# DylanAuty/ObjCAViT

Hardware: AMD Instinct MI355X
Metric: images/sec (640x480, bs=16) forward depth inference, 3 batches of 16 in flight per GPU; AbsRel vs CPU ref (higher is better)
Workload: dtype f32 (fp16 / bf16 split contractions)

## Files before the change

include/objcavit_hip.h:

```cpp
#ifndef OBJCAVIT_HIP_H
#define OBJCAVIT_HIP_H

#include <stddef.h>
#include <stdint.h>

#ifdef __cplusplus
extern "C" {
#endif

typedef void* ocv_stream_t;

#define OCV_ABI_VERSION 5
int ocv_abi_version(void);
const char* ocv_last_error(void);

int ocv_range_flag_set(unsigned* flag);
int ocv_range_flag_take_fwd(unsigned* flag, unsigned* out, ocv_stream_t stream);
int ocv_attention_set_fp32_range(int on);
int ocv_attention_set_dispatch(int form);

#define OCV_ACT_NONE 0
#define OCV_ACT_RELU 1
#define OCV_ACT_LEAKY_RELU 2
#define OCV_ACT_SILU 3
// ... 133 lines not shown
int ocv_pointwise_conv_nhwc_split_ws_fwd(const float* x, const float* gate, int rows_per_image, const void* w_packed,
                                         const float* bias, const float* residual, float* y, void* y_hl, long M, int Cin, int Cout,
                                         int act, void* workspace, size_t workspace_bytes, ocv_stream_t stream);
int ocv_pointwise_hl_set_dispatch(int rt, int tn);
int ocv_pointwise_hl_fwd(const void* x_hl, int Cin, const void* w_packed, long w_image_elems, int rows_per_image,
                         const float* bias, const float* residual, float* y, void* y_hl, long M, int Cout, int act,
                         ocv_stream_t stream);
int ocv_stem_conv_fwd(const float* x, const float* w, const float* bias, float* y, int B, int Cin, int H, int W, int Cout,
                      int k, int stride, int pad_t, int pad_l, int Ho, int Wo, int act, ocv_stream_t stream);
int ocv_depthwise_conv_nhwc_fwd(const float* in, const float* w, const float* bias, float* out, int B, int C, int H,
                                int W, int k, int stride, int pad_t, int pad_l, int Ho, int Wo, int act,
                                ocv_stream_t stream);
int ocv_depthwise_set_dispatch(int mode);
int ocv_depthwise_sum_tiles(int B, int C, int Ho, int Wo, int k, int stride);
int ocv_depthwise_conv_nhwc_sum_fwd(const float* in, const float* w, const float* bias, float* out, float* part, int B,
                                    int C, int H, int W, int k, int stride, int pad_t, int pad_l, int Ho, int Wo,
                                    ocv_stream_t stream);
int ocv_se_gate_partials_fwd(const float* part, int tiles, long pixels_per_image, const float* w1, const float* b1,
                             const float* w2t, const float* b2, float* gate, float* hidden_ws, int B, int C, int R,
                             ocv_stream_t stream);
int ocv_depthwise_conv_nhwc_sum_hl_fwd(const float* in, const float* w, const float* bias, float* out, void* out_hl, float* part,
                                       int B, int C, int H, int W, int k, int stride, int pad_t, int pad_l, int Ho, int Wo,
                                       ocv_stream_t stream);
int ocv_se_gate_weights_fwd(const float* part, int tiles, long pixels_per_image, const float* w1, const float* b1,
                            const float* w2t, const float* b2, const float* W, void* w_packed, long w_image_elems, float* gate,
                            float* hidden_ws, int B, int C, int R, int N, ocv_stream_t stream);


size_t ocv_channel_mean_workspace_bytes(int B, int C, long P);
int ocv_channel_mean_nhwc_fwd(const float* x, float* out, int B, int C, long P, void* workspace, size_t workspace_bytes,
                              ocv_stream_t stream);

int ocv_se_gate_fwd(const float* mean, const float* w1, const float* b1, const float* w2t, const float* b2, float* gate,
                    float* hidden_ws, int B, int C, int R, ocv_stream_t stream);

int ocv_conv_nhwc_fwd(const float* x1, int C1, const float* x2, int C2, const void* w_hi, const void* w_lo,
                      const float* bias, const float* residual, float* y, int B, int H, int W, int Cout, int ksize,
                      int act, ocv_stream_t stream);
int ocv_conv_nhwc_exact_fwd(const float* x1, int C1, const float* x2, int C2, const float* w_tap_major, const float* bias,
                            const float* residual, float* y, int B, int H, int W, int Cout, int ksize, int act,
                            ocv_stream_t stream);
int ocv_conv3x3_nhwc_strided_fwd(const float* x, int Cin, const void* w_hi, const void* w_lo, const float* bias,
                                 const float* residual, float* y, int B, int H, int W, int Cout, int stride, int pad_t,
                                 int pad_l, int Ho, int Wo, int act, ocv_stream_t stream);

int ocv_mbconv_expand_dw_tiles(int Ho, int Wo, int k, int stride);
// ... 146 lines not shown
```

objcavit_amd/_lib.py:

```python
from __future__ import annotations

import ctypes as C
import os
from typing import Optional

_HERE = os.path.dirname(os.path.abspath(__file__))
LIB_PATH = os.environ.get("OCV_LIB_PATH") or os.path.join(_HERE, "lib", "libobjcavit_hip.so")

_f32p = C.c_void_p
_u8p = C.c_void_p
_stream = C.c_void_p
ABI_VERSION = 5


class EncoderLayerParams(C.Structure):
    _fields_ = [("struct_size", C.c_size_t)] + [(n, C.c_void_p) for n in (
        "in_proj_w", "in_proj_b", "out_proj_w", "out_proj_b", "norm1_w", "norm1_b",
        "linear1_w", "linear1_b", "linear2_w", "linear2_b", "norm2_w", "norm2_b",
        "in_proj_p3", "out_proj_p3", "linear1_p3", "linear2_p3",
        "in_proj_h2", "out_proj_h2", "linear1_h2", "linear2_h2")]

    def __init__(self, *a, **kw):
        super().__init__(*a, **kw)
        self.struct_size = C.sizeof(EncoderLayerParams)
# ... 60 lines not shown
                                          _f32p, C.c_int, C.c_int, C.c_int, C.c_int, _stream]),
    "ocv_patch_embed_workspace_bytes": (C.c_size_t, [C.c_int, C.c_int, C.c_int, C.c_int, C.c_int]),
    "ocv_patch_embed_split_workspace_bytes": (C.c_size_t, [C.c_int, C.c_int, C.c_int, C.c_int, C.c_int]),
    "ocv_patch_embed_split_fwd": (C.c_int, [C.c_void_p, C.c_int, C.c_void_p, C.c_void_p, _f32p, C.c_int, _f32p, _f32p, C.c_long, _f32p, C.c_int,
                                            C.c_int, C.c_int, C.c_int, C.c_void_p, C.c_size_t, _stream]),
    "ocv_patch_embed_fwd": (C.c_int, [_f32p, C.c_int, _f32p, _f32p, _f32p, C.c_long, _f32p, C.c_int, C.c_int, C.c_int, C.c_int,
                                      C.c_int, C.c_void_p, C.c_size_t, _stream]),
    "ocv_pixel_dot_fwd": (C.c_int, [_f32p, C.c_int, _f32p, C.c_long, C.c_int, _f32p, C.c_int, C.c_int, C.c_int, C.c_int, _stream]),
    "ocv_bin_head_workspace_bytes": (C.c_size_t, [C.c_int, C.c_int, C.c_int]),
    "ocv_bin_head_fold_fwd": (C.c_int, [_f32p, C.c_long, C.c_int, _f32p, _f32p, C.c_int, C.c_int, C.c_int, C.c_int, _stream]),
    "ocv_bin_head_folded_fwd": (C.c_int, [_f32p, C.c_int, _f32p, _f32p, _f32p, _f32p, C.c_int, C.c_int, C.c_int, C.c_int, _stream]),
    "ocv_bin_head_partials_bytes": (C.c_size_t, [C.c_int, C.c_int]),
    "ocv_bin_head_folded_ws_fwd": (C.c_int, [_f32p, C.c_int, _f32p, _f32p, _f32p, _f32p, C.c_int, C.c_int, C.c_int, C.c_int,
                                             C.c_void_p, C.c_size_t, _stream]),
    "ocv_bin_head_stats_partials_bytes": (C.c_size_t, [C.c_int, C.c_int]),
    "ocv_bin_head_folded_stats_fwd": (C.c_int, [_f32p, C.c_int, _f32p, _f32p, _f32p, _f32p, C.c_int, C.c_int, C.c_int, C.c_int,
                                                C.c_void_p, C.c_size_t, _f32p, _f32p, _stream]),
    "ocv_bin_head_fwd": (C.c_int, [_f32p, C.c_int, _f32p, C.c_long, C.c_int, _f32p, _f32p, _f32p, _f32p, C.c_int, C.c_int,
                                   C.c_int, C.c_int, C.c_int, C.c_void_p, C.c_size_t, _stream]),
    "ocv_depthwise_conv_fwd": (C.c_int, [_f32p, _f32p, _f32p, _f32p] + [C.c_int] * 11 + [_stream]),
    "ocv_depthwise_set_dispatch": (C.c_int, [C.c_int]),
    "ocv_depthwise_sum_tiles": (C.c_int, [C.c_int] * 6),
    "ocv_depthwise_conv_nhwc_sum_fwd": (C.c_int, [_f32p] * 5 + [C.c_int] * 10 + [_stream]),
    "ocv_se_gate_partials_fwd": (C.c_int, [_f32p, C.c_int, C.c_long, _f32p, _f32p, _f32p, _f32p, _f32p, _f32p, C.c_int,
                                           C.c_int, C.c_int, _stream]),
    "ocv_depth_metrics_workspace_bytes": (C.c_size_t, [C.c_int] * 3),
    "ocv_depth_metrics_fwd": (C.c_int, [_f32p, _f32p, C.c_int, C.c_int, _f32p, C.c_int, C.c_int, C.c_float, C.c_float] + [C.c_int] * 4 +
                              [C.c_long, _f32p, C.c_int, C.c_void_p, C.c_size_t, _stream]),
    "ocv_depth_metrics_loss_workspace_bytes": (C.c_size_t, [C.c_int] * 4),
    "ocv_depth_metrics_loss_fwd": (C.c_int, [_f32p, _f32p, C.c_int, C.c_int, _f32p, C.c_int, C.c_int, C.c_float, C.c_float] + [C.c_int] * 4 +
                                   [_f32p, C.c_int, C.c_long, _f32p, _f32p, C.c_int, C.c_void_p, C.c_size_t, _stream]),
    "ocv_frame_ingest_fwd": (C.c_int, [_u8p, C.c_long, C.c_long, C.c_int, C.c_int, C.c_int, C.c_int, _f32p, _f32p, C.c_int, C.c_int, C.c_int,
                                       C.c_int, C.c_long, _stream]),
    "ocv_depth_ingest_fwd": (C.c_int, [C.c_void_p, C.c_long, C.c_long, C.c_int, C.c_int, C.c_int, C.c_int, C.c_float, _f32p, C.c_int, C.c_int,
                                       C.c_int, _stream]),
    "ocv_frame_resize_supported": (C.c_int, [C.c_int] * 4),
    "ocv_frame_resize_ingest": (C.c_int, [_u8p, C.c_long, C.c_long] + [C.c_int] * 6 + [_f32p, C.c_void_p, _f32p, C.c_int, C.c_void_p, _f32p,
                                          C.c_int, _f32p, C.c_int, C.c_int, C.c_int, C.c_int, C.c_long, _stream]),
    "ocv_frame_ingest_format": (C.c_int, [C.c_int] + [_u8p, C.c_long, C.c_long] * 3 + [C.c_void_p] + [C.c_int] * 4 + [_f32p, _f32p, C.c_int,
                                          C.c_int, C.c_int, C.c_int, C.c_long, _stream]),
    "ocv_frame_resize_ingest_format": (C.c_int, [C.c_int] + [_u8p, C.c_long, C.c_long] * 3 + [C.c_void_p] + [C.c_int] * 6 +
                                       [_f32p, C.c_void_p, _f32p, C.c_int, C.c_void_p, _f32p, C.c_int, _f32p, C.c_int, C.c_int, C.c_int,
                                        C.c_int, C.c_long, _stream]),
    "ocv_frames_to_rgb24": (C.c_int, [C.c_int] + [_u8p, C.c_long, C.c_long] * 3 + [C.c_void_p] + [C.c_int] * 4 + [_u8p, C.c_int, C.c_int,
                                      C.c_int, _stream]),
    "ocv_depth_finalize_fwd": (C.c_int, [_f32p, _f32p, C.c_int, C.c_int, C.c_float, C.c_float, C.c_int, C.c_int, _f32p, C.c_void_p, C.c_float,
# ... 110 lines not shown
```

objcavit_amd/build.py:

```python
from __future__ import annotations

import os
import shutil
import subprocess
import sys

HERE = os.path.dirname(os.path.abspath(__file__))
CSRC = os.environ.get("OCV_CSRC_DIR") or os.path.join(HERE, "csrc")
LIB_DIR = os.path.join(HERE, "lib")
LIB_PATH = os.path.join(LIB_DIR, "libobjcavit_hip.so")
SOURCES = ("capi.hip", "linear.hip", "attention.hip", "patch_embed.hip", "bin_head.hip", "depthwise.hip", "conv_igemm.hip", "conv_dma.hip", "conv_winograd.hip", "encoder_nhwc.hip", "upsample.hip", "pointwise_split.hip", "stem.hip", "depthwise_se.hip", "se_gate.hip", "metrics.hip", "mbconv_fused.hip", "pos_sample.hip", "conv_exact.hip", "token_split3.hip", "xattn_split3.hip", "token_pack.hip", "tap_interp.hip", "pointwise_hl.hip", "xattn_h2.hip", "conv_few.hip", "token_h2.hip", "objects_pad.hip", "bin_edges.hip", "frame_ingest.hip", "frame_resize.hip", "depth_finalize.hip", "object_depth.hip", "point_cloud.hip", "surface_normals.hip", "object_metrics.hip", "object_frontend.hip")
ARCH = "gfx950"


def _hipcc() -> str:
    for c in (os.environ.get("HIPCC"), shutil.which("hipcc"), "/opt/rocm/bin/hipcc"):
        if c and os.path.exists(c):
            return c
    raise RuntimeError("hipcc not found")


def _stale() -> bool:
    if not os.path.exists(LIB_PATH):
        return True
    t = os.path.getmtime(LIB_PATH)
    deps = [os.path.join(CSRC, f) for f in os.listdir(CSRC)] + [os.path.join(HERE, "..", "include", "objcavit_hip.h")]
    return any(os.path.getmtime(d) > t for d in deps)


def build(force: bool = False, verbose: bool = False, out: str = None) -> str:
    out = out or os.environ.get("OCV_LIB_OUT")
    if out:
        return _build_to(os.path.abspath(out), os.path.abspath(out) + ".objs", verbose)
    if not force and not _stale():
# ... 39 lines not shown
```

objcavit_amd/csrc/depthwise_se.hip:

```cpp
#include <stdlib.h>

#include "mbconv_tile.hpp"

namespace {

struct DWSArgs {
  const float *in, *w, *bias;
  float *out, *part;
  __bf16* out_hl;
  int C, H, W, Ho, Wo, pad_t, pad_l;
  int QL, PL, RY;
  int wox, nwork, tiles, chunks;
};

template <int K, int S, int PX>
__global__ __launch_bounds__(256, 2) void dw_slide_kernel(DWSArgs p) {
  constexpr int NIN = (PX - 1) * S + K;
  constexpr bool WLDS = K > 3;
  __shared__ float4 red[256];
  __shared__ float4 wsh[WLDS ? K * K * 64 : 1];
  const int tid = threadIdx.x;
  const int q = tid % p.QL, pl = tid / p.QL;
  const int c4n = p.C >> 2;
  int tile, chunk;
// ... 335 lines not shown
template <int S, int QLP>
int launch_dwr(const DWRArgs& a, int B, hipStream_t st) {
  ocv_allow_dynamic_lds<dw_rows_kernel<S, QLP>>();
  constexpr size_t lds = DWRShape<S, QLP>::LDS;
  hipLaunchKernelGGL((dw_rows_kernel<S, QLP>), dim3((unsigned)((long)a.tiles * a.chunks * B)), dim3(dwr_threads(S)), lds, st, a);
  OCV_CHECK_LAUNCH("ocv_depthwise_conv_nhwc_sum_fwd(rows)");
  return 0;
}

}

extern "C" int ocv_depthwise_set_dispatch(int mode) {
  OCV_CHECK_ARG(mode >= 0 && mode <= 2, "ocv_depthwise_set_dispatch: mode must be 0 (automatic), 1 (register window) or 2 (LDS rows), got %d", mode);
  dw_dispatch() = mode;
  return 0;
}

extern "C" int ocv_depthwise_sum_tiles(int B, int C, int Ho, int Wo, int k, int stride) {
  if (B < 1 || C < 4 || C % 4 != 0 || Ho < 1 || Wo < 1 || (k != 3 && k != 5) || (stride != 1 && stride != 2)) return 0;
  if (dw_use_rows(C, Ho, Wo, k, stride)) return dwr_geom(B, C, Ho, Wo, stride).tiles;
  return dws_geom(B, C, Ho, Wo, k, stride).tiles;
}

extern "C" int ocv_depthwise_conv_nhwc_sum_fwd(const float* in, const float* w, const float* bias, float* out, float* part,
                                               int B, int C, int H, int W, int k, int stride, int pad_t, int pad_l,
                                               int Ho, int Wo, ocv_stream_t stream) {
  return ocv_depthwise_conv_nhwc_sum_hl_fwd(in, w, bias, out, nullptr, part, B, C, H, W, k, stride, pad_t, pad_l, Ho, Wo, stream);
}

extern "C" int ocv_depthwise_conv_nhwc_sum_hl_fwd(const float* in, const float* w, const float* bias, float* out, void* out_hl,
                                                  float* part, int B, int C, int H, int W, int k, int stride, int pad_t,
                                                  int pad_l, int Ho, int Wo, ocv_stream_t stream) {
  OCV_CHECK_ARG(in && w && (out || out_hl) && part, "ocv_depthwise_conv_nhwc_sum_fwd: null pointer");
  OCV_CHECK_ARG(out_hl == nullptr || (C % 32 == 0 && ocv_aligned16(out_hl)), "ocv_depthwise_conv_nhwc_sum_hl_fwd: the split output needs C to be a multiple of 32 (got %d) and 16-byte alignment", C);
  if (ocv_check_dw_geometry("ocv_depthwise_conv_nhwc_sum_fwd", true, B, C, H, W, k, stride, pad_t, pad_l, Ho, Wo,
                            ocv_aligned16(in) && ocv_aligned16(w) && ocv_aligned16(out) && ocv_aligned16(bias) && ocv_aligned16(part)) != 0)
    return -1;
  hipStream_t st = (hipStream_t)stream;
  if (dw_use_rows(C, Ho, Wo, k, stride)) {
    const DWRGeom r = dwr_geom(B, C, Ho, Wo, stride);
    OCV_CHECK_ARG((long)r.tiles * r.chunks * B < (1L << 31), "ocv_depthwise_conv_nhwc_sum_fwd: too many workgroups");
    OCV_CHECK_ARG((long)W * C < (1L << 31), "ocv_depthwise_conv_nhwc_sum_fwd: input rows of 2^31 elements or more");
    DWRArgs a{in, w, bias, out, part, (__bf16*)out_hl, C, H, W, Ho, Wo, pad_t, pad_l, r.QL, r.TH, r.nxt, r.tiles, r.chunks};
    if (stride == 1) return r.QLP == 32 ? launch_dwr<1, 32>(a, B, st) : launch_dwr<1, 16>(a, B, st);
    return r.QLP == 32 ? launch_dwr<2, 32>(a, B, st) : launch_dwr<2, 16>(a, B, st);
  }
  const DWSGeom g = dws_geom(B, C, Ho, Wo, k, stride);
  OCV_CHECK_ARG((long)g.tiles * g.chunks * B < (1L << 31), "ocv_depthwise_conv_nhwc_sum_fwd: too many workgroups");
  DWSArgs a{in, w, bias, out, part, (__bf16*)out_hl, C, H, W, Ho, Wo, pad_t, pad_l, g.QL, g.PL, g.RY, g.wox, g.nwork, g.tiles, g.chunks};
  if (k == 3 && stride == 1) return launch_dws<3, 1, 4>(a, g, B, st);
  if (k == 3 && stride == 2) return launch_dws<3, 2, 2>(a, g, B, st);
  if (k == 5 && stride == 1) return launch_dws<5, 1, 2>(a, g, B, st);
  return launch_dws<5, 2, 1>(a, g, B, st);
}
```

objcavit_amd/csrc/mbconv_tile.hpp:

```cpp
#pragma once
#include "common.hpp"
#include "lds_dma.hpp"

typedef __bf16 bf16x8 __attribute__((ext_vector_type(8)));
typedef __bf16 bf16x4 __attribute__((ext_vector_type(4)));

__device__ __forceinline__ bf16x8 ldb8(const __bf16* p) { return *reinterpret_cast<const bf16x8*>(p); }

__device__ __forceinline__ float4 mul4(float4 a, const float4 g) {
  a.x *= g.x; a.y *= g.y; a.z *= g.z; a.w *= g.w;
  return a;
}
__device__ __forceinline__ float4 fma4(const float4 w, const float4 v, float4 a) {
  a.x = fmaf(w.x, v.x, a.x); a.y = fmaf(w.y, v.y, a.y); a.z = fmaf(w.z, v.z, a.z); a.w = fmaf(w.w, v.w, a.w);
  return a;
}
__device__ __forceinline__ float4 silu4(float4 r) {
  r.x = fast_silu(r.x); r.y = fast_silu(r.y); r.z = fast_silu(r.z); r.w = fast_silu(r.w);
  return r;
}

__device__ __forceinline__ void split8(const float4 u, const float4 v, bf16x8& hi, bf16x8& lo) {
  const float f[8] = {u.x, u.y, u.z, u.w, v.x, v.y, v.z, v.w};
#pragma unroll
// ... 9 lines not shown
#pragma unroll
  for (int e = 0; e < 4; ++e) {
    const __bf16 h = (__bf16)f[e];
    hi[e] = h;
    lo[e] = (__bf16)(f[e] - (float)h);
  }
}

__device__ __forceinline__ f32x16 mfma3(const bf16x8 ah, const bf16x8 al, const bf16x8 bh, const bf16x8 bl, f32x16 acc) {
  acc = __builtin_amdgcn_mfma_f32_32x32x16_bf16(ah, bh, acc, 0, 0, 0);
  acc = __builtin_amdgcn_mfma_f32_32x32x16_bf16(ah, bl, acc, 0, 0, 0);
  acc = __builtin_amdgcn_mfma_f32_32x32x16_bf16(al, bh, acc, 0, 0, 0);
  return acc;
}

template <class T>
__device__ __forceinline__ T* w_frag(T* wp, int jt, int Kp, int s, int lane) {
  return wp + (((long)jt * (Kp >> 4) + s) * 2) * 512 + lane * 8;
}

constexpr int TS = 32;
constexpr int TSCRATCH = 32 * TS;

__device__ __forceinline__ void dw_xcd_decode(int tiles, int chunks, int& tile, int& chunk, long& b) {
  const int wg = ocv_xcd_remap(blockIdx.x, gridDim.x);
  tile = wg % tiles;
  const int rest = wg / tiles;
  chunk = rest % chunks;
  b = rest / chunks;
}

template <auto Kernel>
inline void ocv_allow_dynamic_lds(int bytes = 160 * 1024) {
  static const hipError_t once = hipFuncSetAttribute((const void*)Kernel, hipFuncAttributeMaxDynamicSharedMemorySize, bytes);
  (void)once;
}

inline int ocv_check_dw_geometry(const char* name, bool quad_channels, int B, int C, int H, int W, int k, int stride, int pad_t,
                                 int pad_l, int Ho, int Wo, bool aligned) {
  const bool sizes = B >= 1 && H >= 1 && W >= 1 && Ho >= 1 && Wo >= 1;
  if (quad_channels)
    OCV_CHECK_ARG(sizes && C >= 4 && C % 4 == 0, "%s: bad sizes (C must be a multiple of 4)", name);
  else
    OCV_CHECK_ARG(sizes, "%s: bad sizes", name);
  OCV_CHECK_ARG((k == 3 || k == 5) && (stride == 1 || stride == 2), "%s: k must be 3 or 5 and stride 1 or 2 (got k=%d s=%d)", name, k, stride);
  OCV_CHECK_ARG(pad_t >= 0 && pad_l >= 0 && pad_t < k && pad_l < k, "%s: bad padding", name);
// ... 5 lines not shown
```

objcavit_amd/csrc/pointwise_split.hip:

```cpp
#include <stdio.h>
#include <stdlib.h>
#include <string.h>

#include "mbconv_tile.hpp"

namespace {

struct PSArgs {
  const float *x, *gate, *bias, *res;
  const __bf16* wp;
  float* y;
  long M;
  int K, Kp, N, rows_per_image, act;
  __bf16* yhl;
  int Cpo;
  int nbx, nby, col_major;
  int ksplit;
};

__device__ __forceinline__ void store_tile(const PSArgs& p, const f32x16& acc, long m_base, int n, int hh) {
  if (n >= p.N) return;
  const float bv = p.bias != nullptr ? p.bias[n] : 0.f;
#pragma unroll
  for (int r = 0; r < 16; ++r) {
    const long m = m_base + acc_row(r, hh);
    if (m < p.M) {
      float v = ocv_act(acc[r] + bv, p.act);
      if (p.res != nullptr) v += p.res[m * p.N + n];
      p.y[m * p.N + n] = v;
    }
  }
}


__device__ __forceinline__ void load_res(const PSArgs& p, float4 (&rq)[4], long m_base, int n0, int lane) {
  const int ncol = n0 + 4 * (lane & 7);
#pragma unroll
  for (int it = 0; it < 4; ++it) {
    const long m = m_base + (lane >> 3) + 8 * it;
    rq[it] = (p.res != nullptr && ncol < p.N && m < p.M) ? ld4(p.res + m * p.N + ncol) : make_float4(0.f, 0.f, 0.f, 0.f);
  }
}

__device__ __forceinline__ void store_tile_lds(const PSArgs& p, const f32x16& acc, float* scratch, const float4* rq,
                                               long m_base, int n0, int lane) {
  const int l31 = lane & 31, hh = lane >> 5;
  if ((p.N & 3) != 0) {
    store_tile(p, acc, m_base, n0 + l31, hh);
    return;
  }
  const int n = n0 + l31;
  const float bv = (p.bias != nullptr && n < p.N) ? p.bias[n] : 0.f;
#pragma unroll
  for (int r = 0; r < 16; ++r) scratch[acc_row(r, hh) * TS + l31] = ocv_act(acc[r] + bv, p.act);
  const int c4 = lane & 7, ncol = n0 + 4 * c4;
#pragma unroll
  for (int it = 0; it < 4; ++it) {
    const int row = (lane >> 3) + 8 * it;
    const long m = m_base + row;
    float4 v = *reinterpret_cast<const float4*>(scratch + row * TS + 4 * c4);
    if (ncol < p.N && m < p.M) {
      if (rq != nullptr) {
        v.x += rq[it].x; v.y += rq[it].y; v.z += rq[it].z; v.w += rq[it].w;
      } else if (p.res != nullptr) {
        const float4 q = ld4(p.res + m * p.N + ncol);
        v.x += q.x; v.y += q.y; v.z += q.z; v.w += q.w;
      }
      *reinterpret_cast<float4*>(p.y + m * p.N + ncol) = v;
    } else {
      v = make_float4(0.f, 0.f, 0.f, 0.f);
    }
    if (p.yhl != nullptr && ncol < p.Cpo && m < p.M) {
      bf16x4 h, l;
      split4(v, h, l);
      __bf16* d = hl_at(p.yhl, m, ncol, p.Cpo);
      *reinterpret_cast<bf16x4*>(d) = h;
      *reinterpret_cast<bf16x4*>(d + 32) = l;
    }
  }
}

template <int KS>
__global__ __launch_bounds__(256) void pw_rows_kernel(PSArgs p) {
  __shared__ __attribute__((aligned(16))) float tscratch[4 * TSCRATCH];
  const int tid = threadIdx.x, lane = tid & 63, wave = tid >> 6;
  float* scratch = tscratch + wave * TSCRATCH;
  const int l31 = lane & 31, hh = lane >> 5;
  const long m_base = (long)blockIdx.x * 128 + wave * 32;
  const int K = p.K;
  bf16x8 ahi[KS], alo[KS];
  {
    const long m = m_base + l31;
    const bool ok = m < p.M;
    const float* src = p.x + (ok ? m : 0) * K + 8 * hh;
    const float* gsrc = p.gate != nullptr ? p.gate + ((ok ? m : 0) / p.rows_per_image) * K + 8 * hh : nullptr;
#pragma unroll
    for (int s = 0; s < KS; ++s) {
      float4 u = make_float4(0.f, 0.f, 0.f, 0.f), v = u;
      if (ok && 16 * s + 8 * hh < K) {
        u = ld4(src + 16 * s);
        v = ld4(src + 16 * s + 4);
        if (gsrc != nullptr) {
          u = mul4(u, ld4(gsrc + 16 * s));
// ... 411 lines not shown
```

objcavit_amd/hip_ops/encoder.py:

```python
from __future__ import annotations

import ctypes as C
import math
import os
import threading
from typing import Dict, Optional, Sequence, Tuple

import torch

from .. import _lib
from .._lib import EncoderLayerParams, check
from ._core import *
from .conv import *


def depthwise_conv_same(x: torch.Tensor, weight: torch.Tensor, bias: Optional[torch.Tensor], stride: int,
                        act: int = ACT_NONE) -> torch.Tensor:
    lib = _lib.load()
    _req(x, "x"); _req(weight, "weight")
    B, Cc, H, W = x.shape
    k = weight.shape[-1]
    if weight.shape != (Cc, 1, k, k):
        raise ValueError(f"depthwise_conv_same: weight {tuple(weight.shape)} does not match {Cc} channels")
    if bias is not None:
# ... 21 lines not shown

class SplitWeight:

    def __init__(self, weight: torch.Tensor):
        w = weight.detach().float().reshape(weight.shape[0], -1)
        self.cout, self.cin = w.shape
        self.kp = (self.cin + 15) // 16 * 16
        npad = (self.cout + 31) // 32 * 32
        w = torch.nn.functional.pad(w, (0, self.kp - self.cin, 0, npad - self.cout))
        hi = w.to(torch.bfloat16)
        lo = (w - hi.float()).to(torch.bfloat16)
        nt, ns = npad // 32, self.kp // 16
        parts = torch.stack([hi, lo], 0).reshape(2, nt, 32, ns, 2, 8)
        self.packed = parts.permute(1, 3, 0, 4, 2, 5).contiguous().reshape(-1)
        assert self.packed.numel() == nt * ns * 2 * 512


def pointwise_weight(weight: torch.Tensor):
    if os.environ.get("OCV_PW", "split") == "fp32":
        return weight.detach().reshape(weight.shape[0], -1).contiguous()
    return SplitWeight(weight)


def pointwise_nhwc(x: torch.Tensor, weight, bias: Optional[torch.Tensor], act: int = ACT_NONE,
                   gate: Optional[torch.Tensor] = None, residual: Optional[torch.Tensor] = None, out_split: bool = False):
    lib = _lib.load()
    four = x.dim() == 4
    if four:
        x = _nhwc(x, "x")
        B, Cin, H, Wd = x.shape
        M, rpi = B * H * Wd, H * Wd
    else:
        _req(x, "x")
        M, Cin = x.shape
        B, rpi = M, 1
    split = isinstance(weight, SplitWeight)
    if split:
        _req(weight.packed, "weight.packed", torch.bfloat16)
        Cout, wcin = weight.cout, weight.cin
    else:
        w2 = _req(weight.reshape(weight.shape[0], -1), "weight")
        Cout, wcin = w2.shape
    if wcin != Cin:
        raise ValueError(f"pointwise_nhwc: weight with {wcin} input channels does not match {Cin} input channels")
    if bias is not None:
        _req(bias, "bias")
        if bias.numel() != Cout:
            raise ValueError("pointwise_nhwc: bias size mismatch")
# ... 201 lines not shown
        if t is not None:
            _req(t, n)
    R = w1.shape[0]
    if w1.shape != (R, C) or w2t.shape != (R, C) or b1.numel() != R or b2.numel() != C:
        raise ValueError(f"{fn}: {what} shape mismatch")
    if tiles <= 0:
        raise ValueError(f"{fn}: unsupported shape")
    B = x.shape[0]
    part = workspace(B * tiles * C * 4, x.device, "dw_part")
    hid = workspace(B * R * 4, x.device, "se_hidden")
    gate = torch.empty(B, C, dtype=torch.float32, device=x.device) if want_gate else None
    return R, part, hid, gate


def _se_gate_from_partials(lib, part, tiles: int, pixels: int, w1, b1, w2t, b2, gate, hid, R: int):
    B, C = gate.shape
    with timed("se_gate"):
        check(lib.ocv_se_gate_partials_fwd(part.data_ptr(), tiles, pixels, w1.data_ptr(), b1.data_ptr(), w2t.data_ptr(),
                                           b2.data_ptr(), gate.data_ptr(), hid.data_ptr(), B, C, R, _stream()),
              "ocv_se_gate_partials_fwd")


def depthwise_se_gate(x: torch.Tensor, weight_kkc: torch.Tensor, bias: Optional[torch.Tensor], k: int, stride: int,
                      w1: torch.Tensor, b1: torch.Tensor, w2t: torch.Tensor, b2: torch.Tensor, padding: Optional[Tuple[int, int]] = None):
    lib = _lib.load()
    x = _nhwc(x, "x")
    _req(weight_kkc, "weight")
    B, Cc, H, W = x.shape
    if weight_kkc.shape != (k * k, Cc):
        raise ValueError(f"depthwise_se_gate: weight {tuple(weight_kkc.shape)} does not match k={k}, C={Cc}")
    Ho, Wo, pt, pl = _out_pad(H, W, k, stride, padding)
    tiles = lib.ocv_depthwise_sum_tiles(B, Cc, Ho, Wo, k, stride)
    R, part, hid, gate = _se_workspaces("depthwise_se_gate", x, Cc, tiles, w1, b1, w2t, b2, (("bias", bias),))
    out = torch.empty(B, Cc, Ho, Wo, dtype=torch.float32, device=x.device, memory_format=torch.channels_last)
    with timed(f"depthwise|{B},{H},{W},{Cc},k{k}s{stride}"):
        check(lib.ocv_depthwise_conv_nhwc_sum_fwd(x.data_ptr(), weight_kkc.data_ptr(), _ptr(bias), out.data_ptr(),
                                                  part.data_ptr(), B, Cc, H, W, k, stride, pt, pl, Ho, Wo,
                                                  _stream()), "ocv_depthwise_conv_nhwc_sum_fwd")
    _se_gate_from_partials(lib, part, tiles, Ho * Wo, w1, b1, w2t, b2, gate, hid, R)
    return out, gate


def depthwise_se_gate_weights(x: torch.Tensor, weight_kkc: torch.Tensor, bias: Optional[torch.Tensor], k: int, stride: int,
                              w1: torch.Tensor, b1: torch.Tensor, w2t: torch.Tensor, b2: torch.Tensor, w_proj: torch.Tensor,
                              want_gate: bool = False, padding: Optional[Tuple[int, int]] = None):
    lib = _lib.load()
    x = _nhwc(x, "x")
    _req(weight_kkc, "weight")
    B, Cc, H, W = x.shape
    if weight_kkc.shape != (k * k, Cc) or Cc % 32 != 0:
        raise ValueError(f"depthwise_se_gate_weights: weight {tuple(weight_kkc.shape)} does not match k={k}, C={Cc} (C % 32 == 0)")
    Ho, Wo, pt, pl = _out_pad(H, W, k, stride, padding)
    tiles = lib.ocv_depthwise_sum_tiles(B, Cc, Ho, Wo, k, stride)
    R, part, hid, gate = _se_workspaces("depthwise_se_gate_weights", x, Cc, tiles, w1, b1, w2t, b2, (("bias", bias), ("w_proj", w_proj)),
                                        what="parameter", want_gate=want_gate)
    N = w_proj.shape[0]
# ... 80 lines not shown
```

objcavit_amd/modules/efficientnet.py:

```python
from __future__ import annotations

import math

import torch
import torch.nn as nn
import torch.nn.functional as F

from .. import hip_ops

BN_EPS = 1e-3
BN_MOMENTUM = 0.01

B5_STAGES = (("ds", 3, 3, 1, 1, 24), ("ir", 5, 3, 2, 6, 40), ("ir", 5, 5, 2, 6, 64), ("ir", 7, 3, 2, 6, 128),
             ("ir", 7, 5, 1, 6, 176), ("ir", 9, 5, 2, 6, 304), ("ir", 3, 3, 1, 6, 512))
B5_STEM, B5_HEAD = 48, 2048
B1_STAGES = (("ds", 2, 3, 1, 1, 16), ("ir", 3, 3, 2, 6, 24), ("ir", 3, 5, 2, 6, 40), ("ir", 4, 3, 2, 6, 80),
             ("ir", 4, 5, 1, 6, 112), ("ir", 5, 5, 2, 6, 192), ("ir", 2, 3, 1, 6, 320))
B1_STEM, B1_HEAD = 32, 1280


class Conv2dSame(nn.Conv2d):

    def __init__(self, cin, cout, k, stride=1, groups=1, bias=False):
        super().__init__(cin, cout, k, stride=stride, padding=0, groups=groups, bias=bias)
# ... 93 lines not shown


class DepthwiseSeparableConv(_FoldedMixin, nn.Module):
    def __init__(self, cin, cout, k, stride):
        super().__init__()
        self.has_residual = stride == 1 and cin == cout
        self.conv_dw = Conv2dSame(cin, cin, k, stride, groups=cin)
        self.bn1 = _bn(cin)
        self.act1 = nn.SiLU()
        self.se = SqueezeExcite(cin, max(1, int(cin * 0.25)))
        self.conv_pw = nn.Conv2d(cin, cout, 1, bias=False)
        self.bn2 = _bn(cout)
        self.act2 = nn.Identity()

    def _fold(self):
        wd, bd = fold_bn(self.conv_dw, self.bn1)
        wp, bp = fold_bn(self.conv_pw, self.bn2)
        return (_dw_tap_major(wd), bd, hip_ops.pointwise_weight(wp), bp) + _se_params(self.se)

    def forward(self, x):
        if self._fast(x):
            wd, bd, wp, bp, s1, sb1, s2, sb2 = self._folded(x)
            k = self.conv_dw.kernel_size[0]
            y, g = hip_ops.depthwise_se_gate(x, wd, bd, k, self.conv_dw.stride[0], s1, sb1, s2, sb2)
            return hip_ops.pointwise_nhwc(y, wp, bp, hip_ops.ACT_NONE, gate=g, residual=x if self.has_residual else None)
        y = self.act1(self.bn1(self.conv_dw(x)))
        y = self.act2(self.bn2(self.conv_pw(self.se(y))))
        return y + x if self.has_residual else y


class InvertedResidual(_FoldedMixin, nn.Module):
    def __init__(self, cin, cout, k, stride, expand):
        super().__init__()
        mid = cin * expand
        self.has_residual = stride == 1 and cin == cout
        self.conv_pw = nn.Conv2d(cin, mid, 1, bias=False)
        self.bn1 = _bn(mid)
        self.act1 = nn.SiLU()
        self.conv_dw = Conv2dSame(mid, mid, k, stride, groups=mid)
        self.bn2 = _bn(mid)
        self.act2 = nn.SiLU()
        self.se = SqueezeExcite(mid, max(1, int(cin * 0.25)))
        self.conv_pwl = nn.Conv2d(mid, cout, 1, bias=False)
        self.bn3 = _bn(cout)

    def _fold(self):
        we, be = fold_bn(self.conv_pw, self.bn1)
# ... 66 lines not shown
```

Measured before the change: 1132.

## Fuse depthwise conv recompute with gated pointwise projection in DS blocks

For depthwise-separable blocks with small channel counts (Cin==Cout<=32, k=3, stride 1, large spatial size), the depthwise output is no longer written to memory. A pooling-only pass produces the SE partial sums, and a new fused kernel recomputes the depthwise conv row by row and feeds SiLU-gated results straight into the split-bf16 MFMA pointwise projection with bias and residual. This removes a full-resolution activation write and read at the cost of computing the depthwise conv twice. It also adds a new kernel with register-ring prefetching.

```diff
diff --git a/include/objcavit_hip.h b/include/objcavit_hip.h
--- a/include/objcavit_hip.h
+++ b/include/objcavit_hip.h
@@ -179,6 +179,14 @@
 int ocv_depthwise_conv_nhwc_sum_hl_fwd(const float* in, const float* w, const float* bias, float* out, void* out_hl, float* part,
                                        int B, int C, int H, int W, int k, int stride, int pad_t, int pad_l, int Ho, int Wo,
                                        ocv_stream_t stream);
+int ocv_depthwise_pool_nhwc(const float* in, const float* w, const float* bias, float* part, int B, int C, int H, int W, int k,
+                                int stride, int pad_t, int pad_l, int Ho, int Wo, ocv_stream_t stream);
+int ocv_ds_project_set_dispatch(int mode);
+int ocv_ds_project_supported(int Cin, int Cout, int k, int stride);
+int ocv_ds_project_pays(int B, int Cin, int Cout, int Ho, int Wo, int k, int stride);
+int ocv_ds_project_nhwc(const float* x, const float* wd, const float* bd, const float* gate, const void* w_packed,
+                            const float* bias, const float* residual, float* y, int B, int Cin, int Cout, int H, int W, int k,
+                            int stride, int pad_t, int pad_l, int Ho, int Wo, ocv_stream_t stream);
 int ocv_se_gate_weights_fwd(const float* part, int tiles, long pixels_per_image, const float* w1, const float* b1,
                             const float* w2t, const float* b2, const float* W, void* w_packed, long w_image_elems, float* gate,
                             float* hidden_ws, int B, int C, int R, int N, ocv_stream_t stream);
diff --git a/objcavit_amd/_lib.py b/objcavit_amd/_lib.py
--- a/objcavit_amd/_lib.py
+++ b/objcavit_amd/_lib.py
@@ -106,6 +106,11 @@
     "ocv_depthwise_set_dispatch": (C.c_int, [C.c_int]),
     "ocv_depthwise_sum_tiles": (C.c_int, [C.c_int] * 6),
     "ocv_depthwise_conv_nhwc_sum_fwd": (C.c_int, [_f32p] * 5 + [C.c_int] * 10 + [_stream]),
+    "ocv_depthwise_pool_nhwc": (C.c_int, [_f32p] * 4 + [C.c_int] * 10 + [_stream]),
+    "ocv_ds_project_set_dispatch": (C.c_int, [C.c_int]),
+    "ocv_ds_project_supported": (C.c_int, [C.c_int] * 4),
+    "ocv_ds_project_pays": (C.c_int, [C.c_int] * 7),
+    "ocv_ds_project_nhwc": (C.c_int, [_f32p, _f32p, _f32p, _f32p, C.c_void_p, _f32p, _f32p, _f32p] + [C.c_int] * 11 + [_stream]),
     "ocv_se_gate_partials_fwd": (C.c_int, [_f32p, C.c_int, C.c_long, _f32p, _f32p, _f32p, _f32p, _f32p, _f32p, C.c_int,
                                            C.c_int, C.c_int, _stream]),
     "ocv_depth_metrics_workspace_bytes": (C.c_size_t, [C.c_int] * 3),
diff --git a/objcavit_amd/build.py b/objcavit_amd/build.py
--- a/objcavit_amd/build.py
+++ b/objcavit_amd/build.py
@@ -9,7 +9,7 @@
 CSRC = os.environ.get("OCV_CSRC_DIR") or os.path.join(HERE, "csrc")
 LIB_DIR = os.path.join(HERE, "lib")
 LIB_PATH = os.path.join(LIB_DIR, "libobjcavit_hip.so")
-SOURCES = ("capi.hip", "linear.hip", "attention.hip", "patch_embed.hip", "bin_head.hip", "depthwise.hip", "conv_igemm.hip", "conv_dma.hip", "conv_winograd.hip", "encoder_nhwc.hip", "upsample.hip", "pointwise_split.hip", "stem.hip", "depthwise_se.hip", "se_gate.hip", "metrics.hip", "mbconv_fused.hip", "pos_sample.hip", "conv_exact.hip", "token_split3.hip", "xattn_split3.hip", "token_pack.hip", "tap_interp.hip", "pointwise_hl.hip", "xattn_h2.hip", "conv_few.hip", "token_h2.hip", "objects_pad.hip", "bin_edges.hip", "frame_ingest.hip", "frame_resize.hip", "depth_finalize.hip", "object_depth.hip", "point_cloud.hip", "surface_normals.hip", "object_metrics.hip", "object_frontend.hip")
+SOURCES = ("capi.hip", "linear.hip", "attention.hip", "patch_embed.hip", "bin_head.hip", "depthwise.hip", "conv_igemm.hip", "conv_dma.hip", "conv_winograd.hip", "encoder_nhwc.hip", "upsample.hip", "pointwise_split.hip", "stem.hip", "depthwise_se.hip", "ds_project.hip", "se_gate.hip", "metrics.hip", "mbconv_fused.hip", "pos_sample.hip", "conv_exact.hip", "token_split3.hip", "xattn_split3.hip", "token_pack.hip", "tap_interp.hip", "pointwise_hl.hip", "xattn_h2.hip", "conv_few.hip", "token_h2.hip", "objects_pad.hip", "bin_edges.hip", "frame_ingest.hip", "frame_resize.hip", "depth_finalize.hip", "object_depth.hip", "point_cloud.hip", "surface_normals.hip", "object_metrics.hip", "object_frontend.hip")
 ARCH = "gfx950"
 
 
diff --git a/objcavit_amd/csrc/depthwise_se.hip b/objcavit_amd/csrc/depthwise_se.hip
--- a/objcavit_amd/csrc/depthwise_se.hip
+++ b/objcavit_amd/csrc/depthwise_se.hip
@@ -381,6 +381,9 @@
   return dws_geom(B, C, Ho, Wo, k, stride).tiles;
 }
 
+static int dw_sum_launch(const char* name, const float* in, const float* w, const float* bias, float* out, void* out_hl, float* part,
+                         int B, int C, int H, int W, int k, int stride, int pad_t, int pad_l, int Ho, int Wo, ocv_stream_t stream);
+
 extern "C" int ocv_depthwise_conv_nhwc_sum_fwd(const float* in, const float* w, const float* bias, float* out, float* part,
                                                int B, int C, int H, int W, int k, int stride, int pad_t, int pad_l,
                                                int Ho, int Wo, ocv_stream_t stream) {
@@ -392,7 +395,18 @@
                                                   int pad_l, int Ho, int Wo, ocv_stream_t stream) {
   OCV_CHECK_ARG(in && w && (out || out_hl) && part, "ocv_depthwise_conv_nhwc_sum_fwd: null pointer");
   OCV_CHECK_ARG(out_hl == nullptr || (C % 32 == 0 && ocv_aligned16(out_hl)), "ocv_depthwise_conv_nhwc_sum_hl_fwd: the split output needs C to be a multiple of 32 (got %d) and 16-byte alignment", C);
-  if (ocv_check_dw_geometry("ocv_depthwise_conv_nhwc_sum_fwd", true, B, C, H, W, k, stride, pad_t, pad_l, Ho, Wo,
+  return dw_sum_launch("ocv_depthwise_conv_nhwc_sum_fwd", in, w, bias, out, out_hl, part, B, C, H, W, k, stride, pad_t, pad_l, Ho, Wo, stream);
+}
+
+extern "C" int ocv_depthwise_pool_nhwc(const float* in, const float* w, const float* bias, float* part, int B, int C, int H, int W,
+                                           int k, int stride, int pad_t, int pad_l, int Ho, int Wo, ocv_stream_t stream) {
+  OCV_CHECK_ARG(in && w && part, "ocv_depthwise_pool_nhwc: null pointer");
+  return dw_sum_launch("ocv_depthwise_pool_nhwc", in, w, bias, nullptr, nullptr, part, B, C, H, W, k, stride, pad_t, pad_l, Ho, Wo, stream);
+}
+
+static int dw_sum_launch(const char* name, const float* in, const float* w, const float* bias, float* out, void* out_hl, float* part,
+                         int B, int C, int H, int W, int k, int stride, int pad_t, int pad_l, int Ho, int Wo, ocv_stream_t stream) {
+  if (ocv_check_dw_geometry(name, true, B, C, H, W, k, stride, pad_t, pad_l, Ho, Wo,
                             ocv_aligned16(in) && ocv_aligned16(w) && ocv_aligned16(out) && ocv_aligned16(bias) && ocv_aligned16(part)) != 0)
     return -1;
   hipStream_t st = (hipStream_t)stream;
diff --git a/objcavit_amd/csrc/ds_project.hip b/objcavit_amd/csrc/ds_project.hip
--- /dev/null
+++ b/objcavit_amd/csrc/ds_project.hip
@@ -0,0 +1,225 @@
+#include <stdlib.h>
+
+#include <type_traits>
+
+#include "mbconv_tile.hpp"
+
+namespace {
+
+struct DSPArgs {
+  PSArgs ps;
+  const float *wd, *bd;
+  int H, W, Ho, Wo, pad_t, pad_l;
+  int RY, nxb, nruns;
+  long items;
+};
+
+constexpr int DSP_TAPS = 9;
+
+__device__ __forceinline__ void pin4(float4& v) { asm volatile("" : "+v"(v.x), "+v"(v.y), "+v"(v.z), "+v"(v.w)); }
+constexpr int dsp_ring(int ns) { return ns <= 2 ? 2 * ns : ns; }
+
+template <int NS, bool RES>
+__global__ __launch_bounds__(256, 2) void ds_project_kernel(DSPArgs p) {
+  constexpr int Kp = 16 * NS, NU = 2 * NS;
+  constexpr int RING = dsp_ring(NS);
+  constexpr bool WREG = NS <= 2;
+  static_assert(NU % RING == 0 && RING - 1 <= NU, "static ring indices");
+  __shared__ __attribute__((aligned(16))) float tscratch[4 * TSCRATCH];
+  __shared__ __attribute__((aligned(16))) float wtab[(DSP_TAPS + 1) * Kp];
+  __shared__ __attribute__((aligned(16))) float gtab[4 * Kp];
+  const int tid = threadIdx.x, lane = tid & 63, wave = tid >> 6;
+  const int l31 = lane & 31, hh = lane >> 5;
+  const int C = p.ps.K;
+  const long item = (long)ocv_xcd_remap(blockIdx.x, gridDim.x) * 4 + wave;
+  const bool live = item < p.items;
+  const int xb = (int)(item % p.nxb);
+  const long rest = item / p.nxb;
+  const int run = (int)(rest % p.nruns);
+  const long b = rest / p.nruns;
+  for (int i = tid; i < (DSP_TAPS + 1) * Kp; i += 256) {
+    const int t = i / Kp, c = i - t * Kp;
+    float v = 0.f;
+    if (c < C) v = t < DSP_TAPS ? p.wd[t * C + c] : (p.bd != nullptr ? p.bd[c] : 0.f);
+    wtab[i] = v;
+  }
+  if (lane < Kp) gtab[wave * Kp + lane] = (live && lane < C) ? p.ps.gate[b * C + lane] : 0.f;
+  __syncthreads();
+  if (!live) return;
+  const int y0 = run * p.RY, y1 = min(p.Ho, y0 + p.RY);
+  const int ox0 = xb * 32, ox = ox0 + l31;
+  const int ix0 = ox - p.pad_l;
+  bool cok[3];
+#pragma unroll
+  for (int j = 0; j < 3; ++j) cok[j] = ox < p.Wo && ix0 + j >= 0 && ix0 + j < p.W;
+  const float* ib = p.ps.x + b * (long)p.H * p.W * C + 8 * hh;
+  float* scratch = tscratch + wave * TSCRATCH;
+  const float* wt = wtab + 8 * hh;
+  const float* gt = gtab + wave * Kp + 8 * hh;
+  const __bf16* wf = w_frag(p.ps.wp, 0, Kp, 0, lane);
+  const int nt = y1 - y0 + 2;
+
+  float4 in[RING][3];
+  auto load_unit = [&](int t, int u, float4 (&dst)[3]) {
+    const int iy = y0 - p.pad_t + t;
+    const int ch = 4 * u + 4 * (u & ~1);
+    const bool ok = t < nt && iy >= 0 && iy < p.H && ch + 8 * hh < C;
+    const float* src = ib + ((long)iy * p.W + ix0) * C + ch;
+#pragma unroll
+    for (int j = 0; j < 3; ++j) dst[j] = ld4((ok && cok[j]) ? src + j * C : ocv_zero_page);
+  };
+  bf16x8 wh[NS], wl[NS];
+  if (WREG) {
+#pragma unroll
+    for (int s = 0; s < NS; ++s) {
+      wh[s] = ldb8(wf + s * 1024);
+      wl[s] = ldb8(wf + s * 1024 + 512);
+    }
+  }
+#pragma unroll
+  for (int u = 0; u < RING - 1; ++u) load_unit(0, u, in[u]);
+
+  float4 a1[NU], a2[NU];
+#pragma unroll
+  for (int u = 0; u < NU; ++u) a1[u] = a2[u] = make_float4(0.f, 0.f, 0.f, 0.f);
+  const float bv = (p.ps.bias != nullptr && l31 < p.ps.N) ? p.ps.bias[l31] : 0.f;
+  PSArgs q = p.ps;
+  q.act = OCV_ACT_NONE;
+  q.yhl = nullptr;
+  auto input_row = [&](auto emit_tag, int t) {
+    constexpr bool EMIT = decltype(emit_tag)::value;
+    asm volatile("" ::: "memory");
+    const long m_base = (b * p.Ho + (y0 + t - 2)) * (long)p.Wo + ox0;
+    float4 resq[4];
+    if (EMIT) {
+      q.M = m_base - ox0 + p.Wo;
+      if (RES) load_res(q, resq, m_base, 0, lane);
+    }
+    f32x16 acc = {0};
+    float4 fin0;
+#pragma unroll
+    for (int u = 0; u < NU; ++u) {
+      constexpr int AHEAD = RING - 1;
+      if (u + AHEAD < NU) load_unit(t, u + AHEAD, in[(u + AHEAD) % RING]);
+      else load_unit(t + 1, u + AHEAD - NU, in[(u + AHEAD) % RING]);
+      const int s = u >> 1;
+      if (!WREG && EMIT && (u & 1) == 0) {
+        wh[s] = ldb8(wf + s * 1024);
+        wl[s] = ldb8(wf + s * 1024 + 512);
+      }
+      __builtin_amdgcn_sched_barrier(0);
+      const float4(&x3)[3] = in[u % RING];
+      const float* w = wt + 4 * u + 4 * (u & ~1);
+      float4 n1 = *reinterpret_cast<const float4*>(w + DSP_TAPS * Kp), n2 = a1[u], fin = a2[u];
+#pragma unroll
+      for (int j = 0; j < 3; ++j) n1 = fma4(*reinterpret_cast<const float4*>(w + j * Kp), x3[j], n1);
+      __builtin_amdgcn_sched_barrier(0);
+#pragma unroll
+      for (int j = 0; j < 3; ++j) n2 = fma4(*reinterpret_cast<const float4*>(w + (3 + j) * Kp), x3[j], n2);
+      __builtin_amdgcn_sched_barrier(0);
+      pin4(n1);
+      pin4(n2);
+      a1[u] = n1;
+      a2[u] = n2;
+      if (EMIT) {
+#pragma unroll
+        for (int j = 0; j < 3; ++j) fin = fma4(*reinterpret_cast<const float4*>(w + (6 + j) * Kp), x3[j], fin);
+        __builtin_amdgcn_sched_barrier(0);
+        if ((u & 1) == 0) {
+          fin0 = fin;
+        } else {
+          float4 uu = mul4(silu4(fin0), *reinterpret_cast<const float4*>(gt + 16 * s));
+          float4 vv = mul4(silu4(fin), *reinterpret_cast<const float4*>(gt + 16 * s + 4));
+          pin4(uu);
+          pin4(vv);
+          bf16x8 ah, al;
+          split8(uu, vv, ah, al);
+          acc = mfma3(ah, al, wh[s], wl[s], acc);
+        }
+      }
+      __builtin_amdgcn_sched_barrier(0);
+    }
+    if (EMIT) {
+#pragma unroll
+      for (int r = 0; r < 16; ++r) acc[r] = acc[r] + bv;
+      store_tile_lds<false, true>(q, acc, scratch, RES ? resq : nullptr, m_base, 0, lane);
+    }
+  };
+  input_row(std::false_type{}, 0);
+  input_row(std::false_type{}, 1);
+  for (int t = 2; t < nt; ++t) input_row(std::true_type{}, t);
+}
+
+int dsp_rows(int B, int Ho, int Wo) {
+  const long nxb = (Wo + 31) / 32;
+  int ry = 8;
+  while (ry > 2 && (long)B * nxb * ((Ho + ry - 1) / ry) < 4096) ry >>= 1;
+  return ry;
+}
+
+int& dsp_dispatch() {
+  static int mode = 0;
+  return mode;
+}
+
+bool dsp_supported(int Cin, int Cout, int k, int stride) {
+  return k == 3 && stride == 1 && Cin >= 8 && Cin % 8 == 0 && Cin <= 64 && Cout >= 4 && Cout % 4 == 0 && Cout <= 32;
+}
+
+template <int NS>
+int launch_dsp(const DSPArgs& a, hipStream_t st) {
+  const dim3 grid((unsigned)((a.items + 3) / 4));
+  if (a.ps.res != nullptr) hipLaunchKernelGGL((ds_project_kernel<NS, true>), grid, dim3(256), 0, st, a);
+  else hipLaunchKernelGGL((ds_project_kernel<NS, false>), grid, dim3(256), 0, st, a);
+  OCV_CHECK_LAUNCH("ocv_ds_project_nhwc");
+  return 0;
+}
+
+}
+
+extern "C" int ocv_ds_project_set_dispatch(int mode) {
+  OCV_CHECK_ARG(mode >= 0 && mode <= 2, "ocv_ds_project_set_dispatch: mode must be 0 (automatic), 1 (two launches) or 2 (fused), got %d", mode);
+  dsp_dispatch() = mode;
+  return 0;
+}
+
+extern "C" int ocv_ds_project_supported(int Cin, int Cout, int k, int stride) { return dsp_supported(Cin, Cout, k, stride) ? 1 : 0; }
+
+extern "C" int ocv_ds_project_pays(int B, int Cin, int Cout, int Ho, int Wo, int k, int stride) {
+  const int mode = dsp_dispatch();
+  if (mode == 1 || B < 1 || Ho < 1 || Wo < 1 || !dsp_supported(Cin, Cout, k, stride)) return 0;
+  if (mode == 2) return 1;
+  return (Cin == Cout && Cin <= 32 && (long)B * Ho * Wo >= 65536) ? 1 : 0;
+}
+
+extern "C" int ocv_ds_project_nhwc(const float* x, const float* wd, const float* bd, const float* gate, const void* w_packed,
+                                       const float* bias, const float* residual, float* y, int B, int Cin, int Cout, int H, int W,
+                                       int k, int stride, int pad_t, int pad_l, int Ho, int Wo, ocv_stream_t stream) {
+  OCV_CHECK_ARG(x && wd && gate && w_packed && y, "ocv_ds_project_nhwc: null pointer");
+  OCV_CHECK_ARG(dsp_supported(Cin, Cout, k, stride),
+                "ocv_ds_project_nhwc: needs k = 3, stride 1, Cin a multiple of 8 up to 64 and Cout a multiple of 4 up to 32 (got k=%d s=%d Cin=%d Cout=%d)",
+                k, stride, Cin, Cout);
+  if (ocv_check_dw_geometry("ocv_ds_project_nhwc", true, B, Cin, H, W, k, stride, pad_t, pad_l, Ho, Wo,
+                            ocv_aligned16(x) && ocv_aligned16(wd) && ocv_aligned16(bd) && ocv_aligned16(gate) && ocv_aligned16(w_packed) &&
+                                ocv_aligned16(y) && ocv_aligned16(residual)) != 0)
+    return -1;
+  const int Kp = (Cin + 15) / 16 * 16;
+  DSPArgs a{};
+  a.ps = PSArgs{x, gate, bias, residual, (const __bf16*)w_packed, y, (long)B * Ho * Wo, Cin, Kp, Cout, Ho * Wo, OCV_ACT_NONE, nullptr,
+                (Cout + 31) / 32 * 32};
+  a.wd = wd;
+  a.bd = bd;
+  a.H = H; a.W = W; a.Ho = Ho; a.Wo = Wo; a.pad_t = pad_t; a.pad_l = pad_l;
+  a.RY = dsp_rows(B, Ho, Wo);
+  a.nxb = (Wo + 31) / 32;
+  a.nruns = (Ho + a.RY - 1) / a.RY;
+  a.items = (long)B * a.nruns * a.nxb;
+  OCV_CHECK_ARG((a.items + 3) / 4 < (1L << 31), "ocv_ds_project_nhwc: too many workgroups");
+  hipStream_t st = (hipStream_t)stream;
+  switch (Kp / 16) {
+    case 1: return launch_dsp<1>(a, st);
+    case 2: return launch_dsp<2>(a, st);
+    case 3: return launch_dsp<3>(a, st);
+    default: return launch_dsp<4>(a, st);
+  }
+}
diff --git a/objcavit_amd/csrc/mbconv_tile.hpp b/objcavit_amd/csrc/mbconv_tile.hpp
--- a/objcavit_amd/csrc/mbconv_tile.hpp
+++ b/objcavit_amd/csrc/mbconv_tile.hpp
@@ -55,6 +55,81 @@
 constexpr int TS = 32;
 constexpr int TSCRATCH = 32 * TS;
 
+struct PSArgs {
+  const float *x, *gate, *bias, *res;
+  const __bf16* wp;
+  float* y;
+  long M;
+  int K, Kp, N, rows_per_image, act;
+  __bf16* yhl;
+  int Cpo;
+  int nbx, nby, col_major;
+  int ksplit;
+};
+
+__device__ __forceinline__ void store_tile(const PSArgs& p, const f32x16& acc, long m_base, int n, int hh) {
+  if (n >= p.N) return;
+  const float bv = p.bias != nullptr ? p.bias[n] : 0.f;
+#pragma unroll
+  for (int r = 0; r < 16; ++r) {
+    const long m = m_base + acc_row(r, hh);
+    if (m < p.M) {
+      float v = ocv_act(acc[r] + bv, p.act);
+      if (p.res != nullptr) v += p.res[m * p.N + n];
+      p.y[m * p.N + n] = v;
+    }
+  }
+}
+
+
+__device__ __forceinline__ void load_res(const PSArgs& p, float4 (&rq)[4], long m_base, int n0, int lane) {
+  const int ncol = n0 + 4 * (lane & 7);
+#pragma unroll
+  for (int it = 0; it < 4; ++it) {
+    const long m = m_base + (lane >> 3) + 8 * it;
+    rq[it] = (p.res != nullptr && ncol < p.N && m < p.M) ? ld4(p.res + m * p.N + ncol) : make_float4(0.f, 0.f, 0.f, 0.f);
+  }
+}
+
+template <bool RAGGED = true, bool BIASED = false>
+__device__ __forceinline__ void store_tile_lds(const PSArgs& p, const f32x16& acc, float* scratch, const float4* rq,
+                                               long m_base, int n0, int lane) {
+  const int l31 = lane & 31, hh = lane >> 5;
+  if (RAGGED && (p.N & 3) != 0) {
+    store_tile(p, acc, m_base, n0 + l31, hh);
+    return;
+  }
+  const int n = n0 + l31;
+  const float bv = (!BIASED && p.bias != nullptr && n < p.N) ? p.bias[n] : 0.f;
+#pragma unroll
+  for (int r = 0; r < 16; ++r) scratch[acc_row(r, hh) * TS + l31] = ocv_act(BIASED ? acc[r] : acc[r] + bv, p.act);
+  const int c4 = lane & 7, ncol = n0 + 4 * c4;
+#pragma unroll
+  for (int it = 0; it < 4; ++it) {
+    const int row = (lane >> 3) + 8 * it;
+    const long m = m_base + row;
+    float4 v = *reinterpret_cast<const float4*>(scratch + row * TS + 4 * c4);
+    if (ncol < p.N && m < p.M) {
+      if (rq != nullptr) {
+        v.x += rq[it].x; v.y += rq[it].y; v.z += rq[it].z; v.w += rq[it].w;
+      } else if (p.res != nullptr) {
+        const float4 q = ld4(p.res + m * p.N + ncol);
+        v.x += q.x; v.y += q.y; v.z += q.z; v.w += q.w;
+      }
+      *reinterpret_cast<float4*>(p.y + m * p.N + ncol) = v;
+    } else {
+      v = make_float4(0.f, 0.f, 0.f, 0.f);
+    }
+    if (p.yhl != nullptr && ncol < p.Cpo && m < p.M) {
+      bf16x4 h, l;
+      split4(v, h, l);
+      __bf16* d = hl_at(p.yhl, m, ncol, p.Cpo);
+      *reinterpret_cast<bf16x4*>(d) = h;
+      *reinterpret_cast<bf16x4*>(d + 32) = l;
+    }
+  }
+}
+
 __device__ __forceinline__ void dw_xcd_decode(int tiles, int chunks, int& tile, int& chunk, long& b) {
   const int wg = ocv_xcd_remap(blockIdx.x, gridDim.x);
   tile = wg % tiles;
diff --git a/objcavit_amd/csrc/pointwise_split.hip b/objcavit_amd/csrc/pointwise_split.hip
--- a/objcavit_amd/csrc/pointwise_split.hip
+++ b/objcavit_amd/csrc/pointwise_split.hip
@@ -5,80 +5,6 @@
 #include "mbconv_tile.hpp"
 
 namespace {
-
-struct PSArgs {
-  const float *x, *gate, *bias, *res;
-  const __bf16* wp;
-  float* y;
-  long M;
-  int K, Kp, N, rows_per_image, act;
-  __bf16* yhl;
-  int Cpo;
-  int nbx, nby, col_major;
-  int ksplit;
-};
-
-__device__ __forceinline__ void store_tile(const PSArgs& p, const f32x16& acc, long m_base, int n, int hh) {
-  if (n >= p.N) return;
-  const float bv = p.bias != nullptr ? p.bias[n] : 0.f;
-#pragma unroll
-  for (int r = 0; r < 16; ++r) {
-    const long m = m_base + acc_row(r, hh);
-    if (m < p.M) {
-      float v = ocv_act(acc[r] + bv, p.act);
-      if (p.res != nullptr) v += p.res[m * p.N + n];
-      p.y[m * p.N + n] = v;
-    }
-  }
-}
-
-
-__device__ __forceinline__ void load_res(const PSArgs& p, float4 (&rq)[4], long m_base, int n0, int lane) {
-  const int ncol = n0 + 4 * (lane & 7);
-#pragma unroll
-  for (int it = 0; it < 4; ++it) {
-    const long m = m_base + (lane >> 3) + 8 * it;
-    rq[it] = (p.res != nullptr && ncol < p.N && m < p.M) ? ld4(p.res + m * p.N + ncol) : make_float4(0.f, 0.f, 0.f, 0.f);
-  }
-}
-
-__device__ __forceinline__ void store_tile_lds(const PSArgs& p, const f32x16& acc, float* scratch, const float4* rq,
-                                               long m_base, int n0, int lane) {
-  const int l31 = lane & 31, hh = lane >> 5;
-  if ((p.N & 3) != 0) {
-    store_tile(p, acc, m_base, n0 + l31, hh);
-    return;
-  }
-  const int n = n0 + l31;
-  const float bv = (p.bias != nullptr && n < p.N) ? p.bias[n] : 0.f;
-#pragma unroll
-  for (int r = 0; r < 16; ++r) scratch[acc_row(r, hh) * TS + l31] = ocv_act(acc[r] + bv, p.act);
-  const int c4 = lane & 7, ncol = n0 + 4 * c4;
-#pragma unroll
-  for (int it = 0; it < 4; ++it) {
-    const int row = (lane >> 3) + 8 * it;
-    const long m = m_base + row;
-    float4 v = *reinterpret_cast<const float4*>(scratch + row * TS + 4 * c4);
-    if (ncol < p.N && m < p.M) {
-      if (rq != nullptr) {
-        v.x += rq[it].x; v.y += rq[it].y; v.z += rq[it].z; v.w += rq[it].w;
-      } else if (p.res != nullptr) {
-        const float4 q = ld4(p.res + m * p.N + ncol);
-        v.x += q.x; v.y += q.y; v.z += q.z; v.w += q.w;
-      }
-      *reinterpret_cast<float4*>(p.y + m * p.N + ncol) = v;
-    } else {
-      v = make_float4(0.f, 0.f, 0.f, 0.f);
-    }
-    if (p.yhl != nullptr && ncol < p.Cpo && m < p.M) {
-      bf16x4 h, l;
-      split4(v, h, l);
-      __bf16* d = hl_at(p.yhl, m, ncol, p.Cpo);
-      *reinterpret_cast<bf16x4*>(d) = h;
-      *reinterpret_cast<bf16x4*>(d + 32) = l;
-    }
-  }
-}
 
 template <int KS>
 __global__ __launch_bounds__(256) void pw_rows_kernel(PSArgs p) {
diff --git a/objcavit_amd/hip_ops/encoder.py b/objcavit_amd/hip_ops/encoder.py
--- a/objcavit_amd/hip_ops/encoder.py
+++ b/objcavit_amd/hip_ops/encoder.py
@@ -67,8 +67,54 @@
     return SplitWeight(weight)
 
 
+class DeferredDepthwise:
+    __slots__ = ("x", "weight_kkc", "bias", "k", "stride", "pad", "shape")
+
+    def __init__(self, x, weight_kkc, bias, k, stride, pad, shape):
+        self.x, self.weight_kkc, self.bias, self.k, self.stride, self.pad, self.shape = x, weight_kkc, bias, int(k), int(stride), pad, shape
+
+
+def ds_project_pays(B: int, cin: int, weight, H: int, W: int, k: int, stride: int,
+                    padding: Optional[Tuple[int, int]] = None) -> bool:
+    if not isinstance(weight, SplitWeight) or weight.cin != cin:
+        return False
+    Ho, Wo, _, _ = _out_pad(H, W, k, stride, padding)
+    return bool(_lib.load().ocv_ds_project_pays(B, cin, weight.cout, Ho, Wo, k, stride))
+
+
+def _ds_project(d: DeferredDepthwise, weight, bias, act, gate, residual, out_split):
+    lib = _lib.load()
+    if not isinstance(weight, SplitWeight) or act != ACT_NONE or gate is None or out_split:
+        raise ValueError("pointwise_nhwc: a deferred depthwise needs a SplitWeight, a gate, no activation and no split output")
+    B, Cin, Ho, Wo = d.shape
+    _, _, H, W = d.x.shape
+    _req(weight.packed, "weight.packed", torch.bfloat16)
+    Cout = weight.cout
+    if weight.cin != Cin or not lib.ocv_ds_project_supported(Cin, Cout, d.k, d.stride):
+        raise ValueError(f"pointwise_nhwc: deferred depthwise {Cin} -> {Cout}, k={d.k}, stride {d.stride} is not supported")
+    _req(gate, "gate")
+    if gate.shape != (B, Cin):
+        raise ValueError(f"pointwise_nhwc: gate must be {(B, Cin)}, got {tuple(gate.shape)}")
+    if bias is not None:
+        _req(bias, "bias")
+        if bias.numel() != Cout:
+            raise ValueError("pointwise_nhwc: bias size mismatch")
+    y = torch.empty(B, Cout, Ho, Wo, dtype=torch.float32, device=d.x.device, memory_format=torch.channels_last)
+    if residual is not None:
+        residual = _nhwc(residual, "residual")
+        if residual.shape != y.shape:
+            raise ValueError("pointwise_nhwc: residual shape mismatch")
+    with timed(f"ds_project|{B},{H},{W},{Cin},{Cout}"):
+        check(lib.ocv_ds_project_nhwc(d.x.data_ptr(), d.weight_kkc.data_ptr(), _ptr(d.bias), gate.data_ptr(),
+                                          weight.packed.data_ptr(), _ptr(bias), _ptr(residual), y.data_ptr(), B, Cin, Cout, H, W,
+                                          d.k, d.stride, d.pad[0], d.pad[1], Ho, Wo, _stream()), "ocv_ds_project_nhwc")
+    return y
+
+
 def pointwise_nhwc(x: torch.Tensor, weight, bias: Optional[torch.Tensor], act: int = ACT_NONE,
                    gate: Optional[torch.Tensor] = None, residual: Optional[torch.Tensor] = None, out_split: bool = False):
+    if isinstance(x, DeferredDepthwise):
+        return _ds_project(x, weight, bias, act, gate, residual, out_split)
     lib = _lib.load()
     four = x.dim() == 4
     if four:
@@ -316,7 +362,8 @@
 
 
 def depthwise_se_gate(x: torch.Tensor, weight_kkc: torch.Tensor, bias: Optional[torch.Tensor], k: int, stride: int,
-                      w1: torch.Tensor, b1: torch.Tensor, w2t: torch.Tensor, b2: torch.Tensor, padding: Optional[Tuple[int, int]] = None):
+                      w1: torch.Tensor, b1: torch.Tensor, w2t: torch.Tensor, b2: torch.Tensor, padding: Optional[Tuple[int, int]] = None,
+                      defer: bool = False):
     lib = _lib.load()
     x = _nhwc(x, "x")
     _req(weight_kkc, "weight")
@@ -326,6 +373,12 @@
     Ho, Wo, pt, pl = _out_pad(H, W, k, stride, padding)
     tiles = lib.ocv_depthwise_sum_tiles(B, Cc, Ho, Wo, k, stride)
     R, part, hid, gate = _se_workspaces("depthwise_se_gate", x, Cc, tiles, w1, b1, w2t, b2, (("bias", bias),))
+    if defer:
+        with timed(f"depthwise_pool|{B},{H},{W},{Cc},k{k}s{stride}"):
+            check(lib.ocv_depthwise_pool_nhwc(x.data_ptr(), weight_kkc.data_ptr(), _ptr(bias), part.data_ptr(), B, Cc, H, W, k,
+                                                  stride, pt, pl, Ho, Wo, _stream()), "ocv_depthwise_pool_nhwc")
+        _se_gate_from_partials(lib, part, tiles, Ho * Wo, w1, b1, w2t, b2, gate, hid, R)
+        return DeferredDepthwise(x, weight_kkc, bias, k, stride, (pt, pl), (B, Cc, Ho, Wo)), gate
     out = torch.empty(B, Cc, Ho, Wo, dtype=torch.float32, device=x.device, memory_format=torch.channels_last)
     with timed(f"depthwise|{B},{H},{W},{Cc},k{k}s{stride}"):
         check(lib.ocv_depthwise_conv_nhwc_sum_fwd(x.data_ptr(), weight_kkc.data_ptr(), _ptr(bias), out.data_ptr(),
diff --git a/objcavit_amd/modules/efficientnet.py b/objcavit_amd/modules/efficientnet.py
--- a/objcavit_amd/modules/efficientnet.py
+++ b/objcavit_amd/modules/efficientnet.py
@@ -139,7 +139,10 @@
         if self._fast(x):
             wd, bd, wp, bp, s1, sb1, s2, sb2 = self._folded(x)
             k = self.conv_dw.kernel_size[0]
-            y, g = hip_ops.depthwise_se_gate(x, wd, bd, k, self.conv_dw.stride[0], s1, sb1, s2, sb2)
+            s = self.conv_dw.stride[0]
+            defer = hip_ops.ds_project_pays(x.shape[0], x.shape[1], wp, x.shape[2], x.shape[3], k, s)
+            y, g = hip_ops.depthwise_se_gate(x, wd, bd, k, s, s1, sb1, s2, sb2, defer=True) if defer else \
+                hip_ops.depthwise_se_gate(x, wd, bd, k, s, s1, sb1, s2, sb2)
             return hip_ops.pointwise_nhwc(y, wp, bp, hip_ops.ACT_NONE, gate=g, residual=x if self.has_residual else None)
         y = self.act1(self.bn1(self.conv_dw(x)))
         y = self.act2(self.bn2(self.conv_pw(self.se(y))))
```

Result: no change. 1133 (median of 6 runs) (+0.1%).
